# lucidrains/alphafold2

Hardware: AMD Instinct MI355X
Metric: training samples/sec (crop_len=256, msa=128, depth=12) (higher is better)
Workload: dtype bf16; 1 GPU; model=alphafold2 evoformer dim=256 depth=12 heads=8 dim_head=64, global_batch=6, seq_len=256, msa_depth=128, parallelism=dp1

## Files before the change

alphafold2_amd/ops/hip/attention.hip:

```cpp
#include <torch/extension.h>
#include <ATen/hip/HIPContext.h>
#include <ATen/hip/HIPGeneratorImpl.h>
#include <ATen/hip/HIPGraphsUtils.cuh>

#include "attn_dropout.h"
#include "common.h"

typedef __bf16 bf16x8 __attribute__((ext_vector_type(8)));
typedef float f32x4 __attribute__((ext_vector_type(4)));
typedef __bf16 bf16_t;

namespace {

constexpr int BQ = 64;
constexpr int BK = 64;
constexpr int DH = 64;
constexpr int NWAVES = 4;
constexpr int ROWB = DH * sizeof(bf16_t);
constexpr float NEG_INF = -1e30f;

__device__ __forceinline__ int swz(int row, int byte_in_row) {
  return row * ROWB + (byte_in_row ^ ((row & 7) << 4));
}

// ... 1183 lines not shown
    const int c8 = (idx & 7) << 3;
#pragma unroll
    for (int j = 0; j < 8; ++j) tile[c8 + j][row] = acc[pass][j];
  }
  __syncthreads();

  const bool add = accumulate && g * bias_repeat < b0;
  float* out = dbias + ((long)(g * heads + head) * Lq + (long)qtile * BQ) * Lk
      + (long)ktile * BK;
  const int kvc = threadIdx.x & 63;
  for (int qq = threadIdx.x >> 6; qq < q_cols; qq += NWAVES) {
    if (kvc < kv_rows) {
      float* addr = out + (long)qq * Lk + kvc;
      const float val = tile[qq][kvc];
      *addr = add ? *addr + val : val;
    }
  }
}


template <bool HAS_BIAS, bool HAS_MASK>
__global__ __launch_bounds__(256, 4)
void attn_bwd_dv_kernel(TView q, TView k,
                        const bf16_t* __restrict__ bias,
                        const unsigned char* __restrict__ mask,
                        TView dout,
                        const float* __restrict__ lse,
                        TViewMut dv,
                        int Lq, int Lk, int heads, int bias_repeat, int q_repeat,
                        float scale) {
// ... 529 lines not shown
  return keep;
}

std::vector<at::Tensor> attn_bwd(at::Tensor dout, at::Tensor q, at::Tensor k,
                                 at::Tensor v, at::Tensor out, at::Tensor lse,
                                 c10::optional<at::Tensor> bias,
                                 c10::optional<at::Tensor> mask,
                                 long bias_repeat, double scale,
                                 bool need_dbias, long q_repeat,
                                 c10::optional<at::Tensor> dq_out,
                                 c10::optional<at::Tensor> dk_out,
                                 c10::optional<at::Tensor> dv_out,
                                 double dropout_p,
                                 c10::optional<at::Tensor> rng_state,
                                 c10::optional<int64_t> ds_scratch_bytes,
                                 c10::optional<at::Tensor> delta_in) {
  check_qkv_bias(q, k, v, bias, bias_repeat, q_repeat, "attn_bwd");
  const bool has_drop = dropout_p != 0.0;
  BwdDrop<true> dr{};
  if (has_drop) {
    check_dropout_p(dropout_p, "attn_bwd");
    TORCH_CHECK(rng_state.has_value(),
                "attn_bwd: dropout_p > 0 requires the forward's rng_state");
    check_rng_state(*rng_state, q, "attn_bwd");
    dr.state = rng_state->data_ptr<int64_t>();
    dr.thresh = attn_drop::threshold(dropout_p);
    dr.rescale = attn_drop::rescale(dr.thresh);
  }
  const BwdDrop<false> nd{};
  const int B = k.size(0), H = q.size(1), Lq = q.size(2), Lk = k.size(2);
  check_bf16(dout, q, "attn_bwd", "dout");
// ... 52 lines not shown
  static const int64_t ds_scratch_default = [] {
    const char* e = getenv("AF2AMD_DS_SCRATCH_BYTES");
    if (e == nullptr || e[0] == '\0') return (int64_t)2 << 30;
    char* end = nullptr;
    const long long val = strtoll(e, &end, 10);
    TORCH_CHECK(end != e && *end == '\0' && val >= 0,
                "AF2AMD_DS_SCRATCH_BYTES must be a non-negative byte count, "
                "got '", e, "'");
    return (int64_t)val;
  }();
  const int64_t ds_cap = ds_scratch_bytes.value_or(ds_scratch_default);
  TORCH_CHECK(ds_cap >= 0, "attn_bwd: ds_scratch_bytes must be >= 0, got ",
              ds_cap);
  const bool use_ds = need_dbias && ds_cap > 0 && !split_dkv;

  const int n_q = (Lq + BQ - 1) / BQ, n_k = (Lk + BK - 1) / BK;
  const long ds_plane = (long)n_q * BQ * n_k * BK;
  int ds_slice = 0;
  at::Tensor ds_buf;
  if (use_ds) {
    const int64_t per_entry = (int64_t)H * ds_plane * sizeof(bf16_t);
    ds_slice = (int)std::min<int64_t>(
        B, std::max<int64_t>(1, ds_cap / per_entry));
    TORCH_CHECK((long)n_q * BQ <= INT_MAX, "attn_bwd: Lq too large");
    ds_buf = at::empty({(long)ds_slice * H * ds_plane}, q.options());
    TORCH_CHECK(reinterpret_cast<uintptr_t>(ds_buf.data_ptr()) % 16 == 0,
                "attn_bwd: dS scratch must be 16-byte aligned");
    dbias = at::empty({B / bias_repeat, H, Lq, Lk},
                      q.options().dtype(at::kFloat));
  } else if (need_dbias) {
// ... 59 lines not shown
#define DISPATCH_DKV(HB, HM, DB)                                              \
  if (has_drop) DISPATCH_DKV_(HB, HM, DB, true, dr);                          \
  else DISPATCH_DKV_(HB, HM, DB, false, nd)
#define DISPATCH_DKV_(HB, HM, DB, HD, DROP)                                   \
  hipLaunchKernelGGL((attn_bwd_dkv_kernel<HB, HM, DB, HD>), grid_k,           \
      dim3(256), 0, stream, qv, kvv, vv,                                      \
      has_bias ? reinterpret_cast<const bf16_t*>(bias_c.data_ptr()) : nullptr,\
      has_mask ? mask_u8.data_ptr<unsigned char>() : nullptr,                 \
      dov, lse.data_ptr<float>(), delta.data_ptr<float>(), dkv, dvv,          \
      DB == DBIAS_ATOMIC ? dbias.data_ptr<float>() : nullptr,                 \
      dbias_chunks, DB == DBIAS_ATOMIC ? dbias.stride(0) : 0L, dsv,           \
      Lq, Lk, H, (int)bias_repeat, (int)q_repeat, (float)scale, DROP)

  if (use_ds) {
    const int R = (int)bias_repeat;
    for (int b0 = 0; b0 < B; b0 += ds_slice) {
      const int b1 = std::min(B, b0 + ds_slice);
      dsv = DsView{reinterpret_cast<bf16_t*>(ds_buf.data_ptr()), ds_plane,
                   n_q * BQ, b0 * H};
      grid_k = dim3(n_k, (b1 - b0) * H);
      if (has_mask) { DISPATCH_DKV(true, true, DBIAS_STORE); }
      else { DISPATCH_DKV(true, false, DBIAS_STORE); }
      check_launch("attn_bwd_dkv_kernel");
      hipLaunchKernelGGL(attn_bwd_dq_from_ds_kernel,
                         dim3(n_q, (b1 - b0) * H), dim3(256), 0, stream, dsv,
                         kvv, dqv, Lq, Lk, H, (float)scale);
      check_launch("attn_bwd_dq_from_ds_kernel");
      const int g0 = b0 / R, g1 = (b1 - 1) / R;
      hipLaunchKernelGGL(attn_dbias_sum_kernel,
                         dim3(n_q * n_k, (g1 - g0 + 1) * H), dim3(256), 0,
                         stream, dsv, dbias.data_ptr<float>(), Lq, Lk, H, R,
                         b0, b1, g0, b0 > 0 ? 1 : 0);
      check_launch("attn_dbias_sum_kernel");
    }
    return {dq, dk, dv, dbias};
  }

#define DISPATCH_DV(HB, HM)                                                   \
  hipLaunchKernelGGL((attn_bwd_dv_kernel<HB, HM>), grid_k, dim3(256), 0,      \
      stream, qv, kvv,                                                        \
      has_bias ? reinterpret_cast<const bf16_t*>(bias_c.data_ptr()) : nullptr,\
      has_mask ? mask_u8.data_ptr<unsigned char>() : nullptr,                 \
      dov, lse.data_ptr<float>(), dvv,                                        \
      Lq, Lk, H, (int)bias_repeat, (int)q_repeat, (float)scale)

#define DISPATCH_DK(HB, HM, DB)                                               \
  hipLaunchKernelGGL((attn_bwd_dk_kernel<HB, HM, DB>), grid_k, dim3(256), 0,  \
      stream, qv, kvv, vv,                                                    \
      has_bias ? reinterpret_cast<const bf16_t*>(bias_c.data_ptr()) : nullptr,\
// ... 37 lines not shown
```

alphafold2_amd/ops/hip/bindings.cpp:

```cpp
#include <torch/extension.h>

#include <vector>

std::vector<at::Tensor> layernorm_fwd(at::Tensor x, at::Tensor w,
                                      at::Tensor b, double eps);
std::vector<at::Tensor> layernorm_bwd(at::Tensor dy, at::Tensor x,
                                      at::Tensor w, at::Tensor mean,
                                      at::Tensor rstd);
at::Tensor geglu_fwd(at::Tensor x);
at::Tensor geglu_bwd(at::Tensor dy, at::Tensor x);
std::vector<at::Tensor> geglu_bwd_colsum(at::Tensor dy, at::Tensor x);
long geglu_bwd_colsum_max_h();
at::Tensor dist_buckets(at::Tensor coords, at::Tensor boundaries);
at::Tensor pcgemm(at::Tensor A, at::Tensor B, long Bb, long M, long N,
                  long K, long D,
                  long a_bs, long a_ms, long a_ks,
                  long b_bs, long b_ns, long b_ks, double alpha,
                  long variant);
at::Tensor gatemul_fwd(at::Tensor x, at::Tensor g, long xs, long gs,
                       c10::optional<at::Tensor> rowmask);
std::vector<at::Tensor> gatemul_bwd(at::Tensor dy, at::Tensor x, at::Tensor g,
                                    long xs, long gs,
                                    c10::optional<at::Tensor> rowmask,
                                    c10::optional<at::Tensor> dx_out,
// ... 33 lines not shown
    c10::optional<at::Tensor> mask, bool need_dedges);
long se3_core_max_n(long heads, long dim_head, long edge_dim);
std::vector<at::Tensor> egnn_core_fwd(
    at::Tensor P, at::Tensor Q, at::Tensor x, at::Tensor edges,
    at::Tensor W_e, at::Tensor w_d, at::Tensor W2, at::Tensor b2,
    at::Tensor Wc1, at::Tensor bc1, at::Tensor Wc2, at::Tensor bc2,
    double eps, c10::optional<at::Tensor> mask);
std::vector<at::Tensor> egnn_core_bwd(
    at::Tensor dm, at::Tensor ddx, at::Tensor P, at::Tensor Q, at::Tensor x,
    at::Tensor edges, at::Tensor W_e, at::Tensor w_d, at::Tensor W2,
    at::Tensor b2, at::Tensor Wc1, at::Tensor bc1, at::Tensor Wc2,
    at::Tensor bc2, double eps, c10::optional<at::Tensor> mask);
long egnn_core_max_edge_dim();
at::Tensor pairrep_fwd(at::Tensor left, at::Tensor right, at::Tensor emb,
                       at::Tensor rel);
std::vector<at::Tensor> attn_fwd(at::Tensor q, at::Tensor k, at::Tensor v,
                                 c10::optional<at::Tensor> bias,
                                 c10::optional<at::Tensor> mask,
                                 long bias_repeat, double scale,
                                 long q_repeat, double dropout_p,
                                 c10::optional<at::Tensor> rng_state);
at::Tensor attn_dropout_mask(at::Tensor rng_state, long B, long H, long Lq,
                             long Lk, double dropout_p);
std::vector<at::Tensor> attn_bwd(at::Tensor dout, at::Tensor q, at::Tensor k,
                                 at::Tensor v, at::Tensor out, at::Tensor lse,
                                 c10::optional<at::Tensor> bias,
                                 c10::optional<at::Tensor> mask,
                                 long bias_repeat, double scale,
                                 bool need_dbias, long q_repeat,
                                 c10::optional<at::Tensor> dq_out,
                                 c10::optional<at::Tensor> dk_out,
                                 c10::optional<at::Tensor> dv_out,
                                 double dropout_p,
                                 c10::optional<at::Tensor> rng_state,
                                 c10::optional<int64_t> ds_scratch_bytes,
                                 c10::optional<at::Tensor> delta);
std::vector<at::Tensor> attn_gate_bwd(at::Tensor dy, at::Tensor out,
                                      at::Tensor g, at::Tensor dg_out,
                                      bool want_colsum);
std::vector<at::Tensor> tplattn_fwd(at::Tensor q, at::Tensor kv, long heads,
                                    c10::optional<at::Tensor> key_mask,
                                    c10::optional<at::Tensor> query_mask);
std::vector<at::Tensor> tplattn_bwd(at::Tensor dout, at::Tensor q,
                                    at::Tensor kv, at::Tensor out,
                                    at::Tensor lse, long heads,
                                    c10::optional<at::Tensor> key_mask,
                                    c10::optional<at::Tensor> query_mask);

PYBIND11_MODULE(TORCH_EXTENSION_NAME, m) {
  m.def("layernorm_fwd", &layernorm_fwd, "fused LayerNorm forward (gfx950)");
  m.def("layernorm_bwd", &layernorm_bwd, "fused LayerNorm backward (gfx950)");
// ... 21 lines not shown
        py::arg("gs"), py::arg("rowmask") = c10::nullopt,
        py::arg("dx_out") = c10::nullopt, py::arg("dg_out") = c10::nullopt,
        py::arg("dxs") = 0, py::arg("dgs") = 0);
  m.def("linear_fwd", &linear_fwd,
        "tall-M small-K linear GEMM, bias/residual epilogue (gfx950 MFMA)",
        py::arg("x"), py::arg("W"), py::arg("bias") = c10::nullopt,
        py::arg("resid") = c10::nullopt, py::arg("stage") = -1);
  m.def("ff1_geglu_fwd", &ff1_geglu_fwd,
        "linear GEMM with fused GEGLU epilogue (gfx950 MFMA)",
        py::arg("x"), py::arg("W"), py::arg("bias") = c10::nullopt,
        py::arg("stage") = -1, py::arg("want_inter") = true);
  m.def("pairrep_fwd", &pairrep_fwd,
        "fused pair-rep build: outer sum + rel-pos embedding gather "
        "(gfx950, K13)", py::arg("left"), py::arg("right"), py::arg("emb"),
        py::arg("rel"));
  m.def("ipa_core_fwd", &ipa_core_fwd,
        "fused fp32 IPA attention core forward -> [out, attn, gpts]; attn "
        "and gpts are saved for the backward only with save_stats "
        "(gfx950, K7)",
        py::arg("q_s"), py::arg("k_s"), py::arg("v_s"), py::arg("q_pg"),
        py::arg("k_pg"), py::arg("v_pg"), py::arg("bias"), py::arg("pair"),
        py::arg("rot"), py::arg("trans"), py::arg("point_w"),
        py::arg("scale_s"), py::arg("scale_b"), py::arg("scale_p"),
        py::arg("eps"), py::arg("mask") = c10::nullopt,
        py::arg("save_stats") = false);
  m.def("ipa_core_bwd", &ipa_core_bwd,
        "fused fp32 IPA attention core backward: gradients of the eleven "
        "core inputs, row-side + column-side kernels, no atomics "
        "(gfx950, K7)",
        py::arg("dout"), py::arg("attn"), py::arg("gpts"), py::arg("q_s"),
// ... 64 lines not shown
        py::arg("q_repeat") = 1, py::arg("dropout_p") = 0.0,
        py::arg("rng_state") = c10::nullopt);
  m.def("attn_dropout_mask", &attn_dropout_mask,
        "keep mask (B, H, Lq, Lk) uint8 of the fused attention dropout",
        py::arg("rng_state"), py::arg("B"), py::arg("H"), py::arg("Lq"),
        py::arg("Lk"), py::arg("dropout_p"));
  m.def("attn_bwd", &attn_bwd, "fused flash attention backward (gfx950)",
        py::arg("dout"), py::arg("q"), py::arg("k"), py::arg("v"),
        py::arg("out"), py::arg("lse"), py::arg("bias"), py::arg("mask"),
        py::arg("bias_repeat"), py::arg("scale"), py::arg("need_dbias"),
        py::arg("q_repeat") = 1,
        py::arg("dq_out") = c10::nullopt, py::arg("dk_out") = c10::nullopt,
        py::arg("dv_out") = c10::nullopt, py::arg("dropout_p") = 0.0,
        py::arg("rng_state") = c10::nullopt,
        py::arg("ds_scratch_bytes") = c10::nullopt,
        py::arg("delta") = c10::nullopt);
  m.def("attn_gate_bwd", &attn_gate_bwd,
        "gate backward of gated attention in one pass -> [dO, delta"
        "[, colsum]]; dg goes into dg_out, a slice of the packed gradient "
        "(gfx950)",
        py::arg("dy"), py::arg("out"), py::arg("g"), py::arg("dg_out"),
        py::arg("want_colsum") = false);
  m.def("tplattn_fwd", &tplattn_fwd,
        "template pointwise attention forward, one query and T keys per "
        "pair position, operands in their projection layouts -> [out, lse] "
        "(gfx950, bf16 / fp32, K5)",
        py::arg("q"), py::arg("kv"), py::arg("heads"),
        py::arg("key_mask") = c10::nullopt,
        py::arg("query_mask") = c10::nullopt);
  m.def("tplattn_bwd", &tplattn_bwd,
        "template pointwise attention backward -> [dq, dkv]; dkv is one "
// ... 7 lines not shown
```

alphafold2_amd/ops/hip/colsum.h:

```cpp
#pragma once

#include <map>
#include <mutex>
#include <utility>

#include <ATen/hip/HIPContext.h>
#include <hip/hip_runtime.h>

constexpr int COLSUM_MAX_BLOCKS = 2048;

inline long colsum_grid(const void* kernel, int block, long blocks_needed) {
  static std::mutex mu;
  static std::map<std::pair<const void*, int>, long> cache;
  int dev = 0;
  C10_HIP_CHECK(hipGetDevice(&dev));
  long resident;
  {
    std::lock_guard<std::mutex> lock(mu);
    const auto key = std::make_pair(kernel, dev);
    auto it = cache.find(key);
    if (it == cache.end()) {
      int per_cu = 0;
      C10_HIP_CHECK(hipOccupancyMaxActiveBlocksPerMultiprocessor(
          &per_cu, kernel, block, 0));
      const long cus = at::cuda::getDeviceProperties(dev)->multiProcessorCount;
      it = cache.emplace(key, (per_cu > 0 ? per_cu : 1) * cus).first;
    }
    resident = it->second;
  }
  long grid = blocks_needed < resident ? blocks_needed : resident;
  if (grid > COLSUM_MAX_BLOCKS) grid = COLSUM_MAX_BLOCKS;
  return grid < 1 ? 1 : grid;
}

constexpr int COLSUM_FOLD_THREADS = 1024;

static __global__ __launch_bounds__(COLSUM_FOLD_THREADS)
void colsum_fold_kernel(const float* __restrict__ part,
                               float* __restrict__ out, int nb, int C) {
  __shared__ float sh[64][17];
  const int cl = threadIdx.x & 15;
  const int r = threadIdx.x >> 4;
  const int c = blockIdx.x * 16 + cl;
  float s = 0.f;
  if (c < C)
    for (int i = r; i < nb; i += 64) s += part[(long)i * C + c];
  sh[r][cl] = s;
  __syncthreads();
  if (r == 0 && c < C) {
    float t = 0.f;
#pragma unroll 8
    for (int j = 0; j < 64; ++j) t += sh[j][cl];
    out[c] = t;
  }
}
```

alphafold2_amd/ops/hip/gatemul.hip:

```cpp
#include <torch/extension.h>
#include <ATen/hip/HIPContext.h>

#include "common.h"
#include "colsum.h"

namespace {

__device__ __forceinline__ float sigmoid_f(float x) {
  return 1.0f / (1.0f + __expf(-x));
}

template <typename T, int VEC, int GROUP, bool RM>
__global__ void gatemul_fwd_kernel(const T* __restrict__ x, long xs,
                                   const T* __restrict__ g, long gs,
                                   const unsigned char* __restrict__ rowmask,
                                   T* __restrict__ y,
                                   long rows, int C) {
  const int RPB = blockDim.x / GROUP;
  const int lane = threadIdx.x % GROUP;
  const int grp = threadIdx.x / GROUP;
  for (long row = (long)blockIdx.x * RPB + grp; row < rows;
       row += (long)gridDim.x * RPB) {
    const T* xr = x + row * xs;
    const T* gr = g + row * gs;
// ... 386 lines not shown
                     reinterpret_cast<const T*>(out.data_ptr()),
                     reinterpret_cast<const T*>(g.data_ptr()), gs,
                     reinterpret_cast<T*>(d_o.data_ptr()),
                     reinterpret_cast<T*>(dg_out.data_ptr()), dgs,
                     delta.data_ptr<float>(),
                     want_colsum ? partials.data_ptr<float>() : nullptr,
                     rows, (int)C, (int)H, (int)L);
  {
    const hipError_t err = hipGetLastError();
    TORCH_CHECK(err == hipSuccess, "attn_gate_bwd: launch failed: ",
                hipGetErrorString(err));
  }

  std::vector<at::Tensor> ret = {d_o.permute({0, 2, 1, 3}), delta};
  if (want_colsum) {
    hipLaunchKernelGGL(colsum_fold_kernel, dim3((C + 15) / 16),
                       dim3(COLSUM_FOLD_THREADS), 0, stream,
                       partials.data_ptr<float>(), colsum.data_ptr<float>(),
                       (int)grid, (int)C);
    ret.push_back(colsum);
  }
  return ret;
}
```

alphafold2_amd/ops/hip/geglu.hip:

```cpp
#include <torch/extension.h>
#include <ATen/hip/HIPContext.h>

#include "common.h"
#include "colsum.h"

namespace {

template <typename T, int VEC>
__global__ void geglu_fwd_kernel(const T* __restrict__ x, T* __restrict__ y,
                                 long rows, int H, int row_shift) {
  const int sub = row_shift ? (threadIdx.x >> row_shift) : 0;
  const int rows_per_iter = row_shift ? (blockDim.x >> row_shift) : 1;
  const int col0 = row_shift
      ? (threadIdx.x & ((1 << row_shift) - 1)) * VEC : threadIdx.x * VEC;
  const int cstep = row_shift ? H : blockDim.x * VEC;
  for (long row = (long)blockIdx.x * rows_per_iter + sub; row < rows;
       row += (long)gridDim.x * rows_per_iter) {
    const T* xr = x + row * (2L * H);
    T* yr = y + row * (long)H;
    for (int col = col0; col < H; col += cstep) {
      T av[VEC], gv[VEC], yv[VEC];
      vload<T, VEC>(xr + col, av);
      vload<T, VEC>(xr + H + col, gv);
#pragma unroll
// ... 221 lines not shown
  if (colt < block && (colt & (colt - 1)) == 0) row_shift = __builtin_ctz(colt);
  const int rpi = row_shift ? block >> row_shift : 1;
  const long grid = colsum_grid(
      reinterpret_cast<const void*>(geglu_bwd_colsum_kernel), block,
      (rows + rpi - 1) / rpi);
  auto fopt = x.options().dtype(at::kFloat);
  auto partials = at::empty({grid, H2}, fopt);
  auto colsum = at::empty({H2}, fopt);
  auto stream = at::cuda::getCurrentHIPStream();
  using T = __hip_bfloat16;
  hipLaunchKernelGGL(geglu_bwd_colsum_kernel, dim3(grid), dim3(block),
                     0, stream, reinterpret_cast<const T*>(dy.data_ptr()),
                     reinterpret_cast<const T*>(x.data_ptr()),
                     reinterpret_cast<T*>(dx.data_ptr()), rows, H, row_shift,
                     partials.data_ptr<float>());
  hipLaunchKernelGGL(colsum_fold_kernel, dim3((H2 + 15) / 16),
                     dim3(COLSUM_FOLD_THREADS), 0, stream,
                     partials.data_ptr<float>(), colsum.data_ptr<float>(),
                     (int)grid, H2);
  return {dx, colsum};
}
```

alphafold2_amd/ops/hip/pairrep.hip:

```cpp
#include <torch/extension.h>
#include <ATen/hip/HIPContext.h>

#include "common.h"

typedef __bf16 bf16x8_t __attribute__((ext_vector_type(8)));
typedef __bf16 pb16;

namespace {

template <typename T>
__global__ void pairrep_fwd_kernel(const T* __restrict__ left,
                                   const T* __restrict__ right,
                                   const T* __restrict__ emb,
                                   const long* __restrict__ rel,
                                   T* __restrict__ out,
                                   int n, int d) {
  extern __shared__ char smem[];
  T* lrow = reinterpret_cast<T*>(smem);
  const long bi = blockIdx.x;
  const long b = bi / n;
  const T* lg = left + bi * (long)d;
  for (int c = threadIdx.x; c < d; c += blockDim.x) lrow[c] = lg[c];
  __syncthreads();

// ... 6 lines not shown
  const int jstep = blockDim.x / chunks;
  for (int j = j0; j < n; j += jstep) {
    const long e = relrow[j];
    T rv[8], ev[8], ov[8];
    vload<T, 8>(rb + (long)j * d + c8, rv);
    vload<T, 8>(emb + e * (long)d + c8, ev);
#pragma unroll
    for (int k = 0; k < 8; ++k) {
      ov[k] = from_f32<T>(to_f32(lrow[c8 + k]) + to_f32(rv[k]) +
                          to_f32(ev[k]));
    }
    vstore<T, 8>(og + (long)j * d + c8, ov);
  }
}

}

at::Tensor pairrep_fwd(at::Tensor left, at::Tensor right, at::Tensor emb,
                       at::Tensor rel) {
  TORCH_CHECK(left.is_contiguous() && right.is_contiguous() &&
              emb.is_contiguous() && rel.is_contiguous(),
              "pairrep_fwd: contiguous inputs required");
  TORCH_CHECK(rel.scalar_type() == at::kLong, "pairrep_fwd: rel must be long");
  const int b = left.size(0), n = left.size(1), d = left.size(2);
  TORCH_CHECK(d % 8 == 0, "pairrep_fwd: d must be a multiple of 8");
  TORCH_CHECK(d <= 2048, "pairrep_fwd: d > 2048 not covered (one block "
              "row owns d/8 chunks across 256 threads)");
  TORCH_CHECK(emb.size(1) == d && right.size(2) == d, "pairrep_fwd: dim");
  auto out = at::empty({b, n, n, d}, left.options());
  const int block = 256;
// ... 19 lines not shown
```

alphafold2_amd/ops/hip/wgrad.hip:

```cpp
#include <torch/extension.h>
#include <ATen/hip/HIPContext.h>

#include <climits>
#include <cstdint>
#include <cstdlib>

#include "colsum.h"
#include "common.h"

typedef __bf16 bf16x8_t __attribute__((ext_vector_type(8)));
typedef float f32x4_t __attribute__((ext_vector_type(4)));
typedef short s16x4_t __attribute__((ext_vector_type(4)));
typedef short s16x8_t __attribute__((ext_vector_type(8)));
typedef __bf16 pb16;

namespace {

constexpr int WM = 128;
constexpr int WN = 128;
constexpr int KS = 64;
constexpr int NT = 256;

constexpr int PR = KS + 8;

// ... 300 lines not shown
  auto stream = at::cuda::getCurrentHIPStream();
  const pb16* a = reinterpret_cast<const pb16*>(dY.data_ptr());
  const pb16* b = reinterpret_cast<const pb16*>(X.data_ptr());
  if (want_cs)
    hipLaunchKernelGGL(wgrad_stream_kernel<true>, dim3((unsigned int)nwg),
                       dim3(SNT), 0, stream, a, b, part.data_ptr<float>(),
                       K, M, N, k_per_slot, ntiles, (int)tiles, nwg, rowlen);
  else
    hipLaunchKernelGGL(wgrad_stream_kernel<false>, dim3((unsigned int)nwg),
                       dim3(SNT), 0, stream, a, b, part.data_ptr<float>(),
                       K, M, N, k_per_slot, ntiles, (int)tiles, nwg, rowlen);
  hipError_t err = hipGetLastError();
  TORCH_CHECK(err == hipSuccess, "wgrad: launch failed: ",
              hipGetErrorString(err));
  if (slots > 1) {
    hipLaunchKernelGGL(colsum_fold_kernel,
                       dim3((unsigned int)((rowlen + 15) / 16)),
                       dim3(COLSUM_FOLD_THREADS), 0, stream,
                       part.data_ptr<float>(), out.data_ptr<float>(),
                       (int)slots, (int)rowlen);
    err = hipGetLastError();
    TORCH_CHECK(err == hipSuccess, "wgrad: fold launch failed: ",
                hipGetErrorString(err));
  }
  std::vector<at::Tensor> ret{out.narrow(0, 0, MN).view({M, N})};
  if (want_cs) ret.push_back(out.narrow(0, MN, M));
  return ret;
}

void wgrad_check(const at::Tensor& dY, const at::Tensor& X) {
  TORCH_CHECK(dY.is_cuda() && X.is_cuda() && dY.device() == X.device(),
              "wgrad: operands must be on one GPU");
  TORCH_CHECK(dY.scalar_type() == at::kBFloat16 &&
              X.scalar_type() == at::kBFloat16, "wgrad: bf16 only");
  TORCH_CHECK(dY.is_contiguous() && X.is_contiguous(),
// ... 60 lines not shown
```

alphafold2_amd/ops/hip_autograd.py:

```python
import torch
from torch.amp import custom_bwd, custom_fwd
from torch.autograd.function import once_differentiable

from .dispatch import _load_ext


class _LayerNormFn(torch.autograd.Function):
    @staticmethod
    def forward(ctx, x, weight, bias, eps):
        ext = _load_ext()
        x = x.contiguous()
        y, mean, rstd = ext.layernorm_fwd(x, weight, bias, float(eps))
        ctx.save_for_backward(x, weight, mean, rstd)
        return y

    @staticmethod
    def backward(ctx, dy):
        ext = _load_ext()
        x, weight, mean, rstd = ctx.saved_tensors
        dx, dw, db = ext.layernorm_bwd(dy.contiguous(), x, weight, mean, rstd)
        return dx, dw, db, None


def hip_layer_norm(x, weight, bias, eps=1e-5):
# ... 754 lines not shown
class _PairRepFn(torch.autograd.Function):

    @staticmethod
    @custom_fwd(device_type='cuda', cast_inputs=torch.bfloat16)
    def forward(ctx, left, right, emb, rel):
        ext = _load_ext()
        ctx.save_for_backward(rel)
        ctx.emb_rows = emb.shape[0]
        return ext.pairrep_fwd(left.contiguous(), right.contiguous(),
                               emb.contiguous(), rel.contiguous())

    @staticmethod
    @custom_bwd(device_type='cuda')
    def backward(ctx, dy):
        (rel,) = ctx.saved_tensors
        d = dy.shape[-1]
        dleft = dy.sum(dim=2)
        dright = dy.sum(dim=1)
        demb = torch.zeros(ctx.emb_rows, d, device=dy.device,
                           dtype=torch.float32)
        demb.index_add_(0, rel.reshape(-1), dy.reshape(-1, d).float())
        return dleft, dright, demb.to(dy.dtype), None


def hip_pair_rep(left, right, emb, rel):
    return _PairRepFn.apply(left, right, emb, rel)


def _byte_mask(mask):
    if mask is None:
        return None
    if mask.dtype not in (torch.bool, torch.uint8):
        mask = mask != 0
    return mask.contiguous()


class _TemplatePointwiseFn(torch.autograd.Function):
# ... 30 lines not shown
```

setup.py:

```python
import os

from setuptools import find_packages, setup

os.environ.setdefault("PYTORCH_ROCM_ARCH", "gfx950")

from torch.utils.cpp_extension import BuildExtension, CUDAExtension

HIP_DIR = os.path.join("alphafold2_amd", "ops", "hip")

ext = CUDAExtension(
    name="alphafold2_amd._hip_ops",
    sources=[
        os.path.join(HIP_DIR, "bindings.cpp"),
        os.path.join(HIP_DIR, "layernorm.hip"),
        os.path.join(HIP_DIR, "geglu.hip"),
        os.path.join(HIP_DIR, "distbucket.hip"),
        os.path.join(HIP_DIR, "attention.hip"),
        os.path.join(HIP_DIR, "gatemul.hip"),
        os.path.join(HIP_DIR, "pcgemm.hip"),
        os.path.join(HIP_DIR, "ffgemm.hip"),
        os.path.join(HIP_DIR, "wgrad.hip"),
        os.path.join(HIP_DIR, "pairrep.hip"),
        os.path.join(HIP_DIR, "ipacore.hip"),
        os.path.join(HIP_DIR, "se3core.hip"),
        os.path.join(HIP_DIR, "egnncore.hip"),
        os.path.join(HIP_DIR, "tplattn.hip"),
    ],
    extra_compile_args={
        "cxx": ["-O3", "-std=c++17"],
        "nvcc": ["-O3", "-std=c++17"],
    },
)

setup(
    name="alphafold2_amd",
    version="0.1.0",
# ... 7 lines not shown
```

Before: 11.86 samples/sec.

## Fuse attention dQ with dBias reduction, add pair-rep backward kernel, vectorize colsum fold

```diff
diff --git a/alphafold2_amd/ops/hip/attention.hip b/alphafold2_amd/ops/hip/attention.hip
--- a/alphafold2_amd/ops/hip/attention.hip
+++ b/alphafold2_amd/ops/hip/attention.hip
@@ -4,6 +4,7 @@
 #include <ATen/hip/HIPGraphsUtils.cuh>
 
 #include "attn_dropout.h"
+#include "colsum.h"
 #include "common.h"
 
 typedef __bf16 bf16x8 __attribute__((ext_vector_type(8)));
@@ -1221,6 +1222,172 @@
       float* addr = out + (long)qq * Lk + kvc;
       const float val = tile[qq][kvc];
       *addr = add ? *addr + val : val;
+    }
+  }
+}
+
+
+__device__ __forceinline__ void ds_sum_add(const float4& v, float* a) {
+  const unsigned int u[4] = {__float_as_uint(v.x), __float_as_uint(v.y),
+                             __float_as_uint(v.z), __float_as_uint(v.w)};
+#pragma unroll
+  for (int i = 0; i < 4; ++i) {
+    a[2 * i] += __uint_as_float(u[i] << 16);
+    a[2 * i + 1] += __uint_as_float(u[i] & 0xffff0000u);
+  }
+}
+
+constexpr int DQ_DBIAS_MAX_NKV = 6;
+
+__device__ __forceinline__ void stage_load_off(const bf16_t* __restrict__ g,
+                                               const unsigned (&off)[2],
+                                               int rows, bool col_ok0,
+                                               bool col_ok1, StageRegs& r) {
+#pragma unroll
+  for (int pass = 0; pass < 2; ++pass) {
+    const int row = (threadIdx.x + pass * 256) >> 3;
+    float4 val = {0, 0, 0, 0};
+    if (row < rows && (pass ? col_ok1 : col_ok0))
+      val = *reinterpret_cast<const float4*>(g + off[pass]);
+    (pass ? r.v1 : r.v0) = val;
+  }
+}
+
+template <int NKV>
+__global__ __launch_bounds__(256, 2)
+void attn_bwd_dq_dbias_kernel(DsView ds, TView k, TViewMut dq,
+                              float* __restrict__ sum_out, long chunk_stride,
+                              int Lq, int Lk, int heads, float scale,
+                              int bias_repeat, int b0, int b1, int g0,
+                              int epb, int direct, int accumulate) {
+  __shared__ __attribute__((aligned(16))) char lds[4][BK * ROWB];
+  static_assert(sizeof(float) * BQ * (BK + 1) <= 4 * BK * ROWB, "tile");
+
+  const int qtile = blockIdx.x;
+  const int gl = blockIdx.y / heads;
+  const int head = blockIdx.y - gl * heads;
+  const int g = g0 + gl;
+  const int r_lo = max(g * bias_repeat, b0);
+  const int r_hi = min((g + 1) * bias_repeat, b1);
+  const int e_lo = r_lo + blockIdx.z * epb;
+  const int e_hi = min(e_lo + epb, r_hi);
+  const int lane = threadIdx.x & 63;
+  const int wave = threadIdx.x >> 6;
+  const int q_rows = min(BQ, Lq - qtile * BQ);
+
+  float sum[NKV][16];
+#pragma unroll
+  for (int t = 0; t < NKV; ++t)
+#pragma unroll
+    for (int j = 0; j < 16; ++j) sum[t][j] = 0.f;
+
+  unsigned ds_off[2], k_off[2];
+  bool col_ok[2];
+#pragma unroll
+  for (int pass = 0; pass < 2; ++pass) {
+    const int idx = threadIdx.x + pass * 256;
+    const int row = idx >> 3;
+    const int c8 = (idx & 7) << 3;
+    ds_off[pass] = (unsigned)row * (unsigned)ds.pitch + c8;
+    k_off[pass] = (unsigned)row * (unsigned)k.rs + c8;
+    col_ok[pass] = c8 < q_rows;
+  }
+
+  StageRegs dsreg, kreg;
+  if (e_lo < e_hi) {
+    stage_load_off(ds.p + ((long)(e_lo - b0) * heads + head) * ds.plane
+                       + qtile * BQ,
+                   ds_off, min(BK, Lk), col_ok[0], col_ok[1], dsreg);
+    stage_load_off(k.base(e_lo, head), k_off, min(BK, Lk), true, true, kreg);
+  }
+  int buf = 0;
+  for (int e = e_lo; e < e_hi; ++e) {
+    const bf16_t* ds_g = ds.p + ((long)(e - b0) * heads + head) * ds.plane
+        + qtile * BQ;
+    const bf16_t* k_g = k.base(e, head);
+    f32x4 dq_acc[4];
+#pragma unroll
+    for (int c = 0; c < 4; ++c) dq_acc[c] = f32x4{0, 0, 0, 0};
+
+#pragma unroll
+    for (int t = 0; t < NKV; ++t) {
+      char* dsl = lds[buf];
+      char* kl = lds[2 + buf];
+      buf ^= 1;
+      stage_store(dsreg, dsl);
+      stage_store(kreg, kl);
+      ds_sum_add(dsreg.v0, sum[t]);
+      ds_sum_add(dsreg.v1, sum[t] + 8);
+      __syncthreads();
+      if (t + 1 < NKV) {
+        const int next_rows = min(BK, Lk - (t + 1) * BK);
+        stage_load_off(ds_g + (long)(t + 1) * BK * ds.pitch, ds_off,
+                       next_rows, col_ok[0], col_ok[1], dsreg);
+        stage_load_off(k_g + (long)(t + 1) * BK * k.rs, k_off, next_rows,
+                       true, true, kreg);
+      } else if (e + 1 < e_hi) {
+        stage_load_off(ds_g + (long)heads * ds.plane, ds_off, min(BK, Lk),
+                       col_ok[0], col_ok[1], dsreg);
+        stage_load_off(k.base(e + 1, head), k_off, min(BK, Lk), true, true,
+                       kreg);
+      }
+
+      bf16x8 ds_frag[2];
+#pragma unroll
+      for (int kblk = 0; kblk < 2; ++kblk)
+        ds_frag[kblk] = frag_tr(dsl, wave * 16, kblk);
+#pragma unroll
+      for (int c = 0; c < 4; ++c) {
+        f32x4 acc = dq_acc[c];
+#pragma unroll
+        for (int kblk = 0; kblk < 2; ++kblk) {
+          bf16x8 kf = frag_tr(kl, c * 16, kblk);
+          acc = __builtin_amdgcn_mfma_f32_16x16x32_bf16(ds_frag[kblk], kf,
+                                                        acc, 0, 0, 0);
+        }
+        dq_acc[c] = acc;
+      }
+    }
+
+    bf16_t* dq_g = dq.base(e, head) + (long)qtile * BQ * dq.rs;
+#pragma unroll
+    for (int reg = 0; reg < 4; ++reg) {
+      const int row = wave * 16 + (lane >> 4) * 4 + reg;
+      if (row < q_rows) {
+#pragma unroll
+        for (int c = 0; c < 4; ++c) {
+          dq_g[(long)row * dq.rs + c * 16 + (lane & 15)] =
+              (bf16_t)(dq_acc[c][reg] * scale);
+        }
+      }
+    }
+  }
+
+  float (*tile)[BK + 1] = reinterpret_cast<float (*)[BK + 1]>(&lds[0][0]);
+  const bool add = direct && accumulate && g * bias_repeat < b0;
+  float* out = sum_out + (long)blockIdx.z * chunk_stride
+      + ((long)((direct ? g : gl) * heads + head) * Lq + (long)qtile * BQ)
+          * Lk;
+  const int kvc = threadIdx.x & 63;
+#pragma unroll
+  for (int t = 0; t < NKV; ++t) {
+    __syncthreads();
+#pragma unroll
+    for (int pass = 0; pass < 2; ++pass) {
+      const int idx = threadIdx.x + pass * 256;
+      const int row = idx >> 3;
+      const int c8 = (idx & 7) << 3;
+#pragma unroll
+      for (int j = 0; j < 8; ++j) tile[c8 + j][row] = sum[t][pass * 8 + j];
+    }
+    __syncthreads();
+    const int kv_rows = min(BK, Lk - t * BK);
+    for (int qq = threadIdx.x >> 6; qq < q_rows; qq += NWAVES) {
+      if (kvc < kv_rows) {
+        float* addr = out + (long)qq * Lk + t * BK + kvc;
+        const float val = tile[qq][kvc];
+        *addr = add ? *addr + val : val;
+      }
     }
   }
 }
@@ -1780,7 +1947,8 @@
                                  double dropout_p,
                                  c10::optional<at::Tensor> rng_state,
                                  c10::optional<int64_t> ds_scratch_bytes,
-                                 c10::optional<at::Tensor> delta_in) {
+                                 c10::optional<at::Tensor> delta_in,
+                                 c10::optional<int64_t> dq_entries_per_block) {
   check_qkv_bias(q, k, v, bias, bias_repeat, q_repeat, "attn_bwd");
   const bool has_drop = dropout_p != 0.0;
   BwdDrop<true> dr{};
@@ -1863,6 +2031,14 @@
               ds_cap);
   const bool use_ds = need_dbias && ds_cap > 0 && !split_dkv;
 
+  static const bool dq_dbias_fused_env = [] {
+    const char* e = getenv("AF2AMD_DQ_DBIAS_FUSED");
+    return !(e != nullptr && e[0] == '0');
+  }();
+  const int64_t epb_arg = dq_entries_per_block.value_or(-1);
+  TORCH_CHECK(!dq_entries_per_block.has_value() || epb_arg >= 0,
+              "attn_bwd: dq_entries_per_block must be >= 0, got ", epb_arg);
+
   const int n_q = (Lq + BQ - 1) / BQ, n_k = (Lk + BK - 1) / BK;
   const long ds_plane = (long)n_q * BQ * n_k * BK;
   int ds_slice = 0;
@@ -1952,6 +2128,28 @@
 
   if (use_ds) {
     const int R = (int)bias_repeat;
+    const long HLL = (long)H * Lq * Lk;
+    const long groups_cap = ((long)ds_slice + R - 1) / R + 1;
+    const bool fused = groups_cap * HLL <= INT_MAX &&
+        (long)BK * n_q * BQ <= INT_MAX && kvv.rs > 0 &&
+        (long)BK * kvv.rs <= INT_MAX &&
+        (dq_entries_per_block.has_value()
+             ? epb_arg != 0 && n_k <= DQ_DBIAS_MAX_NKV
+             : dq_dbias_fused_env && n_k <= 4);
+#define DQ_DBIAS_FOR_NKV(DO)                                                  \
+  switch (n_k) {                                                              \
+    case 1: DO(1); break;                                                     \
+    case 2: DO(2); break;                                                     \
+    case 3: DO(3); break;                                                     \
+    case 4: DO(4); break;                                                     \
+    case 5: DO(5); break;                                                     \
+    default: DO(6); break;                                                    \
+  }
+    const void* fused_kernel = nullptr;
+#define DQ_DBIAS_PTR(NKV)                                                     \
+  fused_kernel = reinterpret_cast<const void*>(&attn_bwd_dq_dbias_kernel<NKV>)
+    DQ_DBIAS_FOR_NKV(DQ_DBIAS_PTR)
+#undef DQ_DBIAS_PTR
     for (int b0 = 0; b0 < B; b0 += ds_slice) {
       const int b1 = std::min(B, b0 + ds_slice);
       dsv = DsView{reinterpret_cast<bf16_t*>(ds_buf.data_ptr()), ds_plane,
@@ -1960,6 +2158,54 @@
       if (has_mask) { DISPATCH_DKV(true, true, DBIAS_STORE); }
       else { DISPATCH_DKV(true, false, DBIAS_STORE); }
       check_launch("attn_bwd_dkv_kernel");
+      if (fused) {
+        const int g0 = b0 / R, g1 = (b1 - 1) / R;
+        const int ng = g1 - g0 + 1;
+        const int span = std::min(R, b1 - b0);
+        long epb = epb_arg;
+        if (epb <= 0) {
+          const long resident = colsum_grid(fused_kernel, 256,
+                                            COLSUM_MAX_BLOCKS);
+          const long chunks = std::max(1L, resident / ((long)n_q * ng * H));
+          epb = (span + chunks - 1) / chunks;
+        }
+        epb = std::min<long>(std::max(1L, epb), span);
+        const int nchunk = (int)((span + epb - 1) / epb);
+        TORCH_CHECK(nchunk <= 65535 && (long)ng * H <= 65535,
+                    "attn_bwd: dQ + dBias grid too large");
+        const bool direct = nchunk == 1;
+        const long C = (long)ng * HLL;
+        at::Tensor part;
+        float* sum_out = dbias.data_ptr<float>();
+        if (!direct) {
+          part = at::empty({nchunk, C}, dbias.options());
+          sum_out = part.data_ptr<float>();
+        }
+#define LAUNCH_DQ_DBIAS(NKV)                                                  \
+  hipLaunchKernelGGL((attn_bwd_dq_dbias_kernel<NKV>),                         \
+                     dim3(n_q, ng * H, nchunk), dim3(256), 0, stream, dsv,    \
+                     kvv, dqv, sum_out, direct ? 0L : C, Lq, Lk, H,           \
+                     (float)scale, R, b0, b1, g0, (int)epb, direct ? 1 : 0,   \
+                     b0 > 0 ? 1 : 0)
+        DQ_DBIAS_FOR_NKV(LAUNCH_DQ_DBIAS)
+#undef LAUNCH_DQ_DBIAS
+        check_launch("attn_bwd_dq_dbias_kernel");
+        if (!direct) {
+          float* dst = dbias.data_ptr<float>() + (long)g0 * HLL;
+          const bool cont = b0 > 0 && (long)g0 * R < b0;
+          if (cont) {
+            colsum_fold_launch(sum_out, dst, nchunk, HLL, true, stream,
+                               false, C);
+            if (ng > 1)
+              colsum_fold_launch(sum_out + HLL, dst + HLL, nchunk, C - HLL,
+                                 false, stream, false, C);
+          } else {
+            colsum_fold_launch(sum_out, dst, nchunk, C, false, stream);
+          }
+          check_launch("colsum_fold (dbias)");
+        }
+        continue;
+      }
       hipLaunchKernelGGL(attn_bwd_dq_from_ds_kernel,
                          dim3(n_q, (b1 - b0) * H), dim3(256), 0, stream, dsv,
                          kvv, dqv, Lq, Lk, H, (float)scale);
@@ -1971,6 +2217,7 @@
                          b0, b1, g0, b0 > 0 ? 1 : 0);
       check_launch("attn_dbias_sum_kernel");
     }
+#undef DQ_DBIAS_FOR_NKV
     return {dq, dk, dv, dbias};
   }
 
diff --git a/alphafold2_amd/ops/hip/bindings.cpp b/alphafold2_amd/ops/hip/bindings.cpp
--- a/alphafold2_amd/ops/hip/bindings.cpp
+++ b/alphafold2_amd/ops/hip/bindings.cpp
@@ -71,6 +71,11 @@
 long egnn_core_max_edge_dim();
 at::Tensor pairrep_fwd(at::Tensor left, at::Tensor right, at::Tensor emb,
                        at::Tensor rel);
+bool pairrep_bwd_covers(at::Tensor dy, long emb_rows);
+std::vector<at::Tensor> pairrep_bwd(at::Tensor dy, at::Tensor rel,
+                                    long emb_rows);
+at::Tensor colsum_fold(at::Tensor part,
+                       c10::optional<at::Tensor> accumulate_into, bool v1);
 std::vector<at::Tensor> attn_fwd(at::Tensor q, at::Tensor k, at::Tensor v,
                                  c10::optional<at::Tensor> bias,
                                  c10::optional<at::Tensor> mask,
@@ -91,7 +96,8 @@
                                  double dropout_p,
                                  c10::optional<at::Tensor> rng_state,
                                  c10::optional<int64_t> ds_scratch_bytes,
-                                 c10::optional<at::Tensor> delta);
+                                 c10::optional<at::Tensor> delta,
+                                 c10::optional<int64_t> dq_entries_per_block);
 std::vector<at::Tensor> attn_gate_bwd(at::Tensor dy, at::Tensor out,
                                       at::Tensor g, at::Tensor dg_out,
                                       bool want_colsum);
@@ -143,6 +149,19 @@
         "fused pair-rep build: outer sum + rel-pos embedding gather "
         "(gfx950, K13)", py::arg("left"), py::arg("right"), py::arg("emb"),
         py::arg("rel"));
+  m.def("pairrep_bwd", &pairrep_bwd,
+        "pair-rep backward from one read of dy -> [dleft, dright, demb], "
+        "fp32 sums rounded once; no atomics (gfx950, K13)",
+        py::arg("dy"), py::arg("rel"), py::arg("emb_rows"));
+  m.def("pairrep_bwd_covers", &pairrep_bwd_covers,
+        "whether pairrep_bwd covers dy's shape, dtype and layout on the "
+        "current device",
+        py::arg("dy"), py::arg("emb_rows"));
+  m.def("colsum_fold", &colsum_fold,
+        "fixed-order fold of (nb, C) fp32 partial rows -> (C,), or added "
+        "into accumulate_into in place; v1 keeps the scalar body",
+        py::arg("part"), py::arg("accumulate_into") = c10::nullopt,
+        py::arg("v1") = false);
   m.def("ipa_core_fwd", &ipa_core_fwd,
         "fused fp32 IPA attention core forward -> [out, attn, gpts]; attn "
         "and gpts are saved for the backward only with save_stats "
@@ -237,7 +256,8 @@
         py::arg("dv_out") = c10::nullopt, py::arg("dropout_p") = 0.0,
         py::arg("rng_state") = c10::nullopt,
         py::arg("ds_scratch_bytes") = c10::nullopt,
-        py::arg("delta") = c10::nullopt);
+        py::arg("delta") = c10::nullopt,
+        py::arg("dq_entries_per_block") = c10::nullopt);
   m.def("attn_gate_bwd", &attn_gate_bwd,
         "gate backward of gated attention in one pass -> [dO, delta"
         "[, colsum]]; dg goes into dg_out, a slice of the packed gradient "
diff --git a/alphafold2_amd/ops/hip/colsum.h b/alphafold2_amd/ops/hip/colsum.h
--- a/alphafold2_amd/ops/hip/colsum.h
+++ b/alphafold2_amd/ops/hip/colsum.h
@@ -1,5 +1,7 @@
 #pragma once
 
+#include <cstdint>
+#include <cstdlib>
 #include <map>
 #include <mutex>
 #include <utility>
@@ -35,22 +37,113 @@
 
 constexpr int COLSUM_FOLD_THREADS = 1024;
 
+template <bool ACC>
 static __global__ __launch_bounds__(COLSUM_FOLD_THREADS)
 void colsum_fold_kernel(const float* __restrict__ part,
-                               float* __restrict__ out, int nb, int C) {
+                        float* __restrict__ out, int nb, int C, long ld) {
   __shared__ float sh[64][17];
   const int cl = threadIdx.x & 15;
   const int r = threadIdx.x >> 4;
   const int c = blockIdx.x * 16 + cl;
   float s = 0.f;
   if (c < C)
-    for (int i = r; i < nb; i += 64) s += part[(long)i * C + c];
+    for (int i = r; i < nb; i += 64) s += part[(long)i * ld + c];
   sh[r][cl] = s;
   __syncthreads();
   if (r == 0 && c < C) {
     float t = 0.f;
 #pragma unroll 8
     for (int j = 0; j < 64; ++j) t += sh[j][cl];
-    out[c] = t;
+    out[c] = ACC ? out[c] + t : t;
   }
 }
+
+template <int CQ, int RL, bool ACC>
+static __global__ __launch_bounds__(CQ * RL)
+void colsum_fold_vec_kernel(const float* __restrict__ part,
+                            float* __restrict__ out, int nb, int C,
+                            long ld) {
+  __shared__ float4 sh[RL][CQ];
+  const int cl = threadIdx.x % CQ;
+  const int r = threadIdx.x / CQ;
+  const int q = blockIdx.x * CQ + cl;
+  const bool ok = q < (C >> 2);
+  float4 s = {0.f, 0.f, 0.f, 0.f};
+  if (ok) {
+    const float* p = part + (long)q * 4;
+    int i = r;
+    for (; i + 7 * RL < nb; i += 8 * RL) {
+      float4 v[8];
+#pragma unroll
+      for (int u = 0; u < 8; ++u)
+        v[u] = *reinterpret_cast<const float4*>(p + (long)(i + u * RL) * ld);
+#pragma unroll
+      for (int u = 0; u < 8; ++u) {
+        s.x += v[u].x; s.y += v[u].y; s.z += v[u].z; s.w += v[u].w;
+      }
+    }
+    for (; i < nb; i += RL) {
+      const float4 v = *reinterpret_cast<const float4*>(p + (long)i * ld);
+      s.x += v.x; s.y += v.y; s.z += v.z; s.w += v.w;
+    }
+  }
+  sh[r][cl] = s;
+  __syncthreads();
+#pragma unroll
+  for (int h = RL / 2; h > 0; h >>= 1) {
+    if (r < h) {
+      const float4 a = sh[r][cl], b = sh[r + h][cl];
+      sh[r][cl] = float4{a.x + b.x, a.y + b.y, a.z + b.z, a.w + b.w};
+    }
+    __syncthreads();
+  }
+  if (r == 0 && ok) {
+    float4 t = sh[0][cl];
+    float4* o = reinterpret_cast<float4*>(out) + q;
+    if (ACC) {
+      const float4 w = *o;
+      t = float4{w.x + t.x, w.y + t.y, w.z + t.z, w.w + t.w};
+    }
+    *o = t;
+  }
+}
+
+inline bool colsum_fold_force_v1() {
+  static const bool v1 = [] {
+    const char* e = getenv("AF2AMD_COLSUM_FOLD_V1");
+    return e != nullptr && e[0] == '1';
+  }();
+  return v1;
+}
+
+inline void colsum_fold_launch(const float* part, float* out, long nb,
+                               long C, bool accumulate, hipStream_t stream,
+                               bool force_v1 = false, long ld = 0) {
+  if (ld == 0) ld = C;
+  const bool vec = !force_v1 && !colsum_fold_force_v1() && C % 4 == 0 &&
+      ld % 4 == 0 &&
+      reinterpret_cast<uintptr_t>(part) % 16 == 0 &&
+      reinterpret_cast<uintptr_t>(out) % 16 == 0;
+#define COLSUM_FOLD_GO(GRID, THREADS, ...)                                  \
+  do {                                                                      \
+    if (accumulate)                                                         \
+      hipLaunchKernelGGL((__VA_ARGS__ true>), dim3((unsigned int)(GRID)),   \
+                         dim3(THREADS), 0, stream, part, out, (int)nb,      \
+                         (int)C, ld);                                       \
+    else                                                                    \
+      hipLaunchKernelGGL((__VA_ARGS__ false>), dim3((unsigned int)(GRID)),  \
+                         dim3(THREADS), 0, stream, part, out, (int)nb,      \
+                         (int)C, ld);                                       \
+  } while (0)
+  if (!vec) {
+    COLSUM_FOLD_GO((C + 15) / 16, COLSUM_FOLD_THREADS, colsum_fold_kernel<);
+    return;
+  }
+  const long quads = C / 4;
+  if (quads >= 16 * 512) {
+    COLSUM_FOLD_GO((quads + 15) / 16, 16 * 16, colsum_fold_vec_kernel<16, 16,);
+  } else {
+    COLSUM_FOLD_GO((quads + 7) / 8, 8 * 128, colsum_fold_vec_kernel<8, 128,);
+  }
+#undef COLSUM_FOLD_GO
+}
diff --git a/alphafold2_amd/ops/hip/colsum.hip b/alphafold2_amd/ops/hip/colsum.hip
--- /dev/null
+++ b/alphafold2_amd/ops/hip/colsum.hip
@@ -0,0 +1,31 @@
+#include <torch/extension.h>
+#include <ATen/hip/HIPContext.h>
+
+#include "colsum.h"
+
+at::Tensor colsum_fold(at::Tensor part,
+                       c10::optional<at::Tensor> accumulate_into, bool v1) {
+  TORCH_CHECK(part.is_cuda() && part.scalar_type() == at::kFloat &&
+              part.is_contiguous() && part.dim() == 2 && part.size(0) >= 1 &&
+              part.size(1) >= 1,
+              "colsum_fold: part must be contiguous fp32 (nb, C)");
+  const long nb = part.size(0), C = part.size(1);
+  TORCH_CHECK(nb <= INT_MAX && C <= INT_MAX, "colsum_fold: nb, C must fit int");
+  at::Tensor out;
+  if (accumulate_into.has_value()) {
+    out = *accumulate_into;
+    TORCH_CHECK(out.is_cuda() && out.device() == part.device() &&
+                out.scalar_type() == at::kFloat && out.is_contiguous() &&
+                out.numel() == C,
+                "colsum_fold: accumulate_into must be contiguous fp32 (C,)");
+  } else {
+    out = at::empty({C}, part.options());
+  }
+  colsum_fold_launch(part.data_ptr<float>(), out.data_ptr<float>(), nb, C,
+                     accumulate_into.has_value(),
+                     at::cuda::getCurrentHIPStream(), v1);
+  const hipError_t err = hipGetLastError();
+  TORCH_CHECK(err == hipSuccess, "colsum_fold: launch failed: ",
+              hipGetErrorString(err));
+  return out;
+}
diff --git a/alphafold2_amd/ops/hip/gatemul.hip b/alphafold2_amd/ops/hip/gatemul.hip
--- a/alphafold2_amd/ops/hip/gatemul.hip
+++ b/alphafold2_amd/ops/hip/gatemul.hip
@@ -424,10 +424,8 @@
 
   std::vector<at::Tensor> ret = {d_o.permute({0, 2, 1, 3}), delta};
   if (want_colsum) {
-    hipLaunchKernelGGL(colsum_fold_kernel, dim3((C + 15) / 16),
-                       dim3(COLSUM_FOLD_THREADS), 0, stream,
-                       partials.data_ptr<float>(), colsum.data_ptr<float>(),
-                       (int)grid, (int)C);
+    colsum_fold_launch(partials.data_ptr<float>(), colsum.data_ptr<float>(),
+                       grid, C, false, stream);
     ret.push_back(colsum);
   }
   return ret;
diff --git a/alphafold2_amd/ops/hip/geglu.hip b/alphafold2_amd/ops/hip/geglu.hip
--- a/alphafold2_amd/ops/hip/geglu.hip
+++ b/alphafold2_amd/ops/hip/geglu.hip
@@ -259,9 +259,7 @@
                      reinterpret_cast<const T*>(x.data_ptr()),
                      reinterpret_cast<T*>(dx.data_ptr()), rows, H, row_shift,
                      partials.data_ptr<float>());
-  hipLaunchKernelGGL(colsum_fold_kernel, dim3((H2 + 15) / 16),
-                     dim3(COLSUM_FOLD_THREADS), 0, stream,
-                     partials.data_ptr<float>(), colsum.data_ptr<float>(),
-                     (int)grid, H2);
+  colsum_fold_launch(partials.data_ptr<float>(), colsum.data_ptr<float>(),
+                     grid, H2, false, stream);
   return {dx, colsum};
 }
diff --git a/alphafold2_amd/ops/hip/pairrep.hip b/alphafold2_amd/ops/hip/pairrep.hip
--- a/alphafold2_amd/ops/hip/pairrep.hip
+++ b/alphafold2_amd/ops/hip/pairrep.hip
@@ -1,6 +1,7 @@
 #include <torch/extension.h>
 #include <ATen/hip/HIPContext.h>
 
+#include "colsum.h"
 #include "common.h"
 
 typedef __bf16 bf16x8_t __attribute__((ext_vector_type(8)));
@@ -44,6 +45,207 @@
   }
 }
 
+constexpr int PB_TILE = 32;
+constexpr int PB_MAX_THREADS = 512;
+
+__device__ __forceinline__ float2 load2f(const float* p) {
+  return *reinterpret_cast<const float2*>(p);
+}
+__device__ __forceinline__ float2 load2f(const __hip_bfloat16* p) {
+  const unsigned int raw = *reinterpret_cast<const unsigned int*>(p);
+  return float2{__uint_as_float(raw << 16),
+                __uint_as_float(raw & 0xffff0000u)};
+}
+__device__ __forceinline__ float2 load2f(const __half* p) {
+  const __half2 h = *reinterpret_cast<const __half2*>(p);
+  return float2{__low2float(h), __high2float(h)};
+}
+
+template <typename T>
+__global__ __launch_bounds__(PB_MAX_THREADS)
+void pairrep_bwd_kernel(const T* __restrict__ dy,
+                        const long* __restrict__ rel,
+                        float* __restrict__ part_lr,
+                        float* __restrict__ part_emb,
+                        int n, int d, int V, long bnd) {
+  extern __shared__ __attribute__((aligned(16))) char smem[];
+  float* tab = reinterpret_cast<float*>(smem);
+  int* rel_l = reinterpret_cast<int*>(smem + (long)V * d * 4);
+
+  const int tj = blockIdx.x, ti = blockIdx.y, bz = blockIdx.z;
+  const int i0 = ti * PB_TILE, j0 = tj * PB_TILE;
+  const int ni = min(PB_TILE, n - i0), nj = min(PB_TILE, n - j0);
+  const int c2 = threadIdx.x * 2;
+  const bool active = c2 < d;
+
+  for (int idx = threadIdx.x; idx < PB_TILE * PB_TILE; idx += blockDim.x) {
+    const int ii = idx >> 5, jj = idx & 31;
+    int e = -1;
+    if (ii < ni && jj < nj) {
+      const long v = rel[((long)bz * n + i0 + ii) * n + j0 + jj];
+      if (v >= 0 && v < V) e = (int)v;
+    }
+    rel_l[idx] = e;
+  }
+  if (active)
+    for (int e = 0; e < V; ++e)
+      *reinterpret_cast<float2*>(tab + (long)e * d + c2) = float2{0.f, 0.f};
+  __syncthreads();
+  if (!active) return;
+
+  float2 dr[PB_TILE];
+#pragma unroll
+  for (int jj = 0; jj < PB_TILE; ++jj) dr[jj] = float2{0.f, 0.f};
+  int cur = -1;
+  float2 eacc = {0.f, 0.f};
+
+  const T* base = dy + (((long)bz * n + i0) * n + j0) * d + c2;
+  float2 nxt[PB_TILE];
+#pragma unroll
+  for (int jj = 0; jj < PB_TILE; ++jj)
+    nxt[jj] = jj < nj ? load2f(base + (long)jj * d) : float2{0.f, 0.f};
+
+  float* pl = part_lr + (long)tj * 2 * bnd + ((long)bz * n + i0) * d + c2;
+  for (int ii = 0; ii < ni; ++ii) {
+    float2 w[PB_TILE];
+#pragma unroll
+    for (int jj = 0; jj < PB_TILE; ++jj) w[jj] = nxt[jj];
+    if (ii + 1 < ni) {
+      const T* row = base + (long)(ii + 1) * n * d;
+#pragma unroll
+      for (int jj = 0; jj < PB_TILE; ++jj)
+        if (jj < nj) nxt[jj] = load2f(row + (long)jj * d);
+    }
+    float2 dl = {0.f, 0.f};
+    const int* rrow = rel_l + ii * PB_TILE;
+#pragma unroll
+    for (int jj = 0; jj < PB_TILE; ++jj) {
+      if (jj < nj) {
+        const float2 f = w[jj];
+        dl.x += f.x; dl.y += f.y;
+        dr[jj].x += f.x; dr[jj].y += f.y;
+        const int e = rrow[jj];
+        if (e != cur) {
+          if (cur >= 0) {
+            float2* t = reinterpret_cast<float2*>(tab + (long)cur * d + c2);
+            const float2 o = *t;
+            *t = float2{o.x + eacc.x, o.y + eacc.y};
+          }
+          cur = e;
+          eacc = float2{0.f, 0.f};
+        }
+        if (e >= 0) { eacc.x += f.x; eacc.y += f.y; }
+      }
+    }
+    *reinterpret_cast<float2*>(pl + (long)ii * d) = dl;
+  }
+  if (cur >= 0) {
+    float2* t = reinterpret_cast<float2*>(tab + (long)cur * d + c2);
+    const float2 o = *t;
+    *t = float2{o.x + eacc.x, o.y + eacc.y};
+  }
+
+  float* pr = part_lr + (long)ti * 2 * bnd + bnd + ((long)bz * n + j0) * d
+      + c2;
+#pragma unroll
+  for (int jj = 0; jj < PB_TILE; ++jj)
+    if (jj < nj) *reinterpret_cast<float2*>(pr + (long)jj * d) = dr[jj];
+
+  const long blk = ((long)bz * gridDim.y + ti) * gridDim.x + tj;
+  float* pe = part_emb + blk * V * d + c2;
+  for (int e = 0; e < V; ++e)
+    *reinterpret_cast<float2*>(pe + (long)e * d) =
+        *reinterpret_cast<const float2*>(tab + (long)e * d + c2);
+}
+
+long pairrep_lds_limit() {
+  int dev = 0, base = 0, optin = 0;
+  C10_HIP_CHECK(hipGetDevice(&dev));
+  C10_HIP_CHECK(hipDeviceGetAttribute(
+      &base, hipDeviceAttributeMaxSharedMemoryPerBlock, dev));
+  if (hipDeviceGetAttribute(&optin, hipDeviceAttributeSharedMemPerBlockOptin,
+                            dev) != hipSuccess) {
+    (void)hipGetLastError();
+    optin = 0;
+  }
+  return base > optin ? base : optin;
+}
+
+long pairrep_bwd_lds_bytes(long V, long d) {
+  return V * d * 4 + PB_TILE * PB_TILE * 4;
+}
+
+}
+
+bool pairrep_bwd_covers(at::Tensor dy, long emb_rows) {
+  if (dy.dim() != 4 || !dy.is_cuda() || !dy.is_contiguous()) return false;
+  const auto st = dy.scalar_type();
+  if (st != at::kBFloat16 && st != at::kFloat && st != at::kHalf)
+    return false;
+  const long b = dy.size(0), n = dy.size(1), d = dy.size(3);
+  if (b < 1 || n < 1 || d < 8 || emb_rows < 1 || dy.size(2) != n)
+    return false;
+  if (d % 8 != 0 || d > 2 * PB_MAX_THREADS || b > 65535) return false;
+  if ((n + PB_TILE - 1) / PB_TILE > 65535) return false;
+  if (2 * b * n * d > INT_MAX || emb_rows * d > INT_MAX) return false;
+  return pairrep_bwd_lds_bytes(emb_rows, d) <= pairrep_lds_limit();
+}
+
+std::vector<at::Tensor> pairrep_bwd(at::Tensor dy, at::Tensor rel,
+                                    long emb_rows) {
+  TORCH_CHECK(pairrep_bwd_covers(dy, emb_rows),
+              "pairrep_bwd: shape, dtype or layout not covered (contiguous "
+              "(b, n, n, d) bf16/fp16/fp32, d % 8 == 0, d <= ",
+              2 * PB_MAX_THREADS, ", the emb_rows x d fp32 table within the "
+              "LDS of a block)");
+  TORCH_CHECK(rel.scalar_type() == at::kLong && rel.is_contiguous() &&
+              rel.is_cuda() && rel.device() == dy.device() &&
+              rel.dim() == 3 && rel.size(0) == dy.size(0) &&
+              rel.size(1) == dy.size(1) && rel.size(2) == dy.size(2),
+              "pairrep_bwd: rel must be contiguous long (b, n, n)");
+  const int b = dy.size(0), n = dy.size(1), d = dy.size(3);
+  const int V = (int)emb_rows;
+  const int T = (n + PB_TILE - 1) / PB_TILE;
+  const long bnd = (long)b * n * d, Vd = (long)V * d;
+  const long tiles = (long)b * T * T;
+  const auto fopt = dy.options().dtype(at::kFloat);
+  auto part_lr = at::empty({T, 2 * bnd}, fopt);
+  auto part_emb = at::empty({tiles, Vd}, fopt);
+  auto out = at::empty({2 * bnd + Vd}, fopt);
+  const int threads = (d / 2 + 63) / 64 * 64;
+  const long smem = pairrep_bwd_lds_bytes(V, d);
+  auto stream = at::cuda::getCurrentHIPStream();
+
+#define LAUNCH(T_)                                                          \
+  do {                                                                      \
+    if (smem > 64 * 1024)                                                   \
+      C10_HIP_CHECK(hipFuncSetAttribute(                                    \
+          reinterpret_cast<const void*>(&pairrep_bwd_kernel<T_>),           \
+          hipFuncAttributeMaxDynamicSharedMemorySize, (int)smem));          \
+    hipLaunchKernelGGL((pairrep_bwd_kernel<T_>), dim3(T, T, b),             \
+                       dim3(threads), smem, stream,                         \
+                       reinterpret_cast<const T_*>(dy.data_ptr()),          \
+                       rel.data_ptr<long>(), part_lr.data_ptr<float>(),     \
+                       part_emb.data_ptr<float>(), n, d, V, bnd);           \
+  } while (0)
+  if (dy.scalar_type() == at::kBFloat16) LAUNCH(__hip_bfloat16);
+  else if (dy.scalar_type() == at::kFloat) LAUNCH(float);
+  else LAUNCH(__half);
+#undef LAUNCH
+  hipError_t err = hipGetLastError();
+  TORCH_CHECK(err == hipSuccess, "pairrep_bwd: launch failed: ",
+              hipGetErrorString(err));
+  float* o = out.data_ptr<float>();
+  colsum_fold_launch(part_lr.data_ptr<float>(), o, T, 2 * bnd, false, stream);
+  colsum_fold_launch(part_emb.data_ptr<float>(), o + 2 * bnd, tiles, Vd,
+                     false, stream);
+  err = hipGetLastError();
+  TORCH_CHECK(err == hipSuccess, "pairrep_bwd: fold launch failed: ",
+              hipGetErrorString(err));
+  auto r = out.to(dy.scalar_type());
+  return {r.narrow(0, 0, bnd).view({b, n, d}),
+          r.narrow(0, bnd, bnd).view({b, n, d}),
+          r.narrow(0, 2 * bnd, Vd).view({V, d})};
 }
 
 at::Tensor pairrep_fwd(at::Tensor left, at::Tensor right, at::Tensor emb,
diff --git a/alphafold2_amd/ops/hip/wgrad.hip b/alphafold2_amd/ops/hip/wgrad.hip
--- a/alphafold2_amd/ops/hip/wgrad.hip
+++ b/alphafold2_amd/ops/hip/wgrad.hip
@@ -338,11 +338,8 @@
   TORCH_CHECK(err == hipSuccess, "wgrad: launch failed: ",
               hipGetErrorString(err));
   if (slots > 1) {
-    hipLaunchKernelGGL(colsum_fold_kernel,
-                       dim3((unsigned int)((rowlen + 15) / 16)),
-                       dim3(COLSUM_FOLD_THREADS), 0, stream,
-                       part.data_ptr<float>(), out.data_ptr<float>(),
-                       (int)slots, (int)rowlen);
+    colsum_fold_launch(part.data_ptr<float>(), out.data_ptr<float>(), slots,
+                       rowlen, false, stream);
     err = hipGetLastError();
     TORCH_CHECK(err == hipSuccess, "wgrad: fold launch failed: ",
                 hipGetErrorString(err));
diff --git a/alphafold2_amd/ops/hip_autograd.py b/alphafold2_amd/ops/hip_autograd.py
--- a/alphafold2_amd/ops/hip_autograd.py
+++ b/alphafold2_amd/ops/hip_autograd.py
@@ -792,13 +792,23 @@
     @custom_bwd(device_type='cuda')
     def backward(ctx, dy):
         (rel,) = ctx.saved_tensors
-        d = dy.shape[-1]
-        dleft = dy.sum(dim=2)
-        dright = dy.sum(dim=1)
-        demb = torch.zeros(ctx.emb_rows, d, device=dy.device,
-                           dtype=torch.float32)
-        demb.index_add_(0, rel.reshape(-1), dy.reshape(-1, d).float())
-        return dleft, dright, demb.to(dy.dtype), None
+        ext = _load_ext()
+        if not _PAIRREP_BWD_V1 and ext.pairrep_bwd_covers(dy, ctx.emb_rows):
+            dleft, dright, demb = ext.pairrep_bwd(dy, rel, ctx.emb_rows)
+            return dleft, dright, demb, None
+        return (*_pairrep_bwd_composed(dy, rel, ctx.emb_rows), None)
+
+
+_PAIRREP_BWD_V1 = _os.environ.get("AF2AMD_PAIRREP_BWD_V1", "0") == "1"
+
+
+def _pairrep_bwd_composed(dy, rel, emb_rows):
+    d = dy.shape[-1]
+    dleft = dy.sum(dim=2)
+    dright = dy.sum(dim=1)
+    demb = torch.zeros(emb_rows, d, device=dy.device, dtype=torch.float32)
+    demb.index_add_(0, rel.reshape(-1), dy.reshape(-1, d).float())
+    return dleft, dright, demb.to(dy.dtype)
 
 
 def hip_pair_rep(left, right, emb, rel):
diff --git a/setup.py b/setup.py
--- a/setup.py
+++ b/setup.py
@@ -20,6 +20,7 @@
         os.path.join(HIP_DIR, "pcgemm.hip"),
         os.path.join(HIP_DIR, "ffgemm.hip"),
         os.path.join(HIP_DIR, "wgrad.hip"),
+        os.path.join(HIP_DIR, "colsum.hip"),
         os.path.join(HIP_DIR, "pairrep.hip"),
         os.path.join(HIP_DIR, "ipacore.hip"),
         os.path.join(HIP_DIR, "se3core.hip"),
```

After: 12.30 samples/sec (median of 6 runs). 3.7% higher.
